# KyleVanMeter/MVOLPS

Measured on AMD Instinct MI355X. Metric: simplex_pivots_per_s, higher is better.
Workload: dtype f64

## Files before the change

### mvolps_amd/csrc/engine.cpp

```cpp
#include <hip/hip_runtime.h>

#include <cmath>
#include <cstdio>
#include <cstdlib>
#include <cstring>
#include <atomic>
#include <functional>
#include <limits>
#include <map>
#include <mutex>
#include <tuple>
#include <unordered_map>
#include <unordered_set>
#include <vector>

#include "engine.hpp"

struct DevMatrix {
  int m0 = 0, n = 0, lda = 0;
  double *plain = nullptr, *packed = nullptr;
  int *len = nullptr;
  std::vector<const void *> rows;
  ~DevMatrix() {
    if (packed && packed != plain) (void)hipFree(packed);
// ... 1033 lines not shown
  if (J.parm.it_lim > 8 && J.try_fused) J.batch = std::min(J.parm.it_lim, 256);
}

static void job_enqueue(Context &c, SolveJob &J) {
  mvx_prob *P = J.P;
  SolveCtx &sc = *J.sc;
  const int m = P->m, n = P->n;
  J.ev_used = 0;
  if (J.mode == SolveJob::FINAL) {
    launch_export(sc.d_ctl, sc.d_stage, m, n, 1, sc.stream);
    stage_copy_async(sc, P);
    return;
  }
  if (J.mode == SolveJob::PHASE1) {
    for (int k = 0; k < J.pb; k++) {
      launch_p1_head(sc.d_ctl, sc.stream);
      launch_p1_fix(sc.d_ctl, n, sc.stream);
      launch_p1_select(sc.d_ctl, sc.stream);
      launch_update(sc.d_ctl, m + 1, n, sc.stream);
    }
    launch_export(sc.d_ctl, sc.d_stage, m, n, 0, sc.stream);
    stage_copy_async(sc, P);
    return;
  }
  const int batch = J.batch;
  if (J.profiled && c.ev_pool.size() < (size_t)2 * batch + 4) {
    size_t old = c.ev_pool.size();
    c.ev_pool.resize((size_t)2 * batch + 4);
    for (size_t k = old; k < c.ev_pool.size(); k++) HIPCHECK(hipEventCreate(&c.ev_pool[k]));
  }
  const int remaining = (J.parm.it_lim >= 0) ? std::max(0, J.parm.it_lim - J.seen_pivots) : (1 << 30);
  auto ev = [&]() {
    if (J.profiled) HIPCHECK(hipEventRecord(c.ev_pool[J.ev_used++], sc.stream));
  };
  int depth;
  if (J.try_fused) depth = std::max(0, std::min(batch, remaining));
  else depth = std::max(1, std::min(batch, remaining));
  auto body = [&](int m_grid) {
    if (J.try_fused) {
      PersistPlan pl;
      if (depth > 0 && !J.profiled && J.resident && !(J.cluster && !g_cluster_broken.load()) && persist_plan(c, P, &pl) && ensure_persist(c, sc, P, pl)) {
        launch_select(sc.d_ctl, sc.stream);
        launch_update(sc.d_ctl, m_grid, n, sc.stream, 1, 1);
        HIPCHECK(hipMemcpyAsync(sc.p_backup, P->slab, P->slab_bytes, hipMemcpyDeviceToDevice, sc.stream));
        HIPCHECK(hipMemcpyAsync(sc.d_pctl, sc.d_ctl, sizeof(Ctl), hipMemcpyDeviceToDevice, sc.stream));
        HIPCHECK(hipMemcpyAsync(sc.d_ppw, sc.d_pw[0], (size_t)P->ld * 8, hipMemcpyDeviceToDevice, sc.stream));
        HIPCHECK(hipMemcpyAsync(sc.d_ppw + P->ld, sc.d_pw[1], (size_t)P->ld * 8, hipMemcpyDeviceToDevice, sc.stream));
        const int head_stride = 4;
        HIPCHECK(hipMemsetAsync(sc.d_pcand, 0, (size_t)2 * pl.nw * head_stride * 8, sc.stream));
        const int steps = 1 << 24;
        if (launch_persist(sc.d_ctl, sc.d_pcand, sc.d_pmsg, sc.d_pabort, (unsigned long long *)(sc.d_pabort + 16), P->m, pl.cpw, pl.nw, sc.p_msg_words, steps, head_stride, sc.stream) == 0) {
          J.persist_queued = true;
          g_persist_launches++;
          launch_select(sc.d_ctl, sc.stream);
          launch_update(sc.d_ctl, m_grid, n, sc.stream, 1, 1);
        } else {
          g_persist_broken = true;
        }
      } else {
        const size_t e_generic = J.ev_used;
        if (J.profiled) J.ev_used += 2;
        if (depth > 0) {
          const bool cl = J.cluster && !g_cluster_broken.load();
          if (!cl) launch_pboot(J.cargs, sc.stream);
          bool first = true;
          const int kc = cl ? std::max(1, std::min(J.chain0, chain_cluster_kmax(m, n))) : std::max(1, J.chain);
          auto chain_launch = [&](int steps) {
            J.cargs.kmax = steps;
            J.cargs.boot = first ? 1 : 0;
            first = false;
            J.cargs.tagbase = sc.xtag;
            sc.xtag += 128;
            if (launch_chain(J.cargs, sc.stream) != 0) g_cluster_broken.store(true);
            g_cluster_launches++;
          };
          for (int left = depth; left > 0;) {
            const int steps = std::min(kc, left);
            if (cl) chain_launch(steps);
            else
              for (int t = 0; t < steps; t++) launch_pstep(J.cargs, t, sc.stream);
            ev();
            launch_fbc3(J.cargs, steps, sc.stream);
            ev();
            launch_fpatch(J.cargs, steps, sc.stream);
            left -= steps;
          }
          if (J.parm.it_lim >= 0 && depth >= remaining && !cl) launch_pc(J.cargs, 0, sc.stream);
        }
        launch_select(sc.d_ctl, sc.stream);
        if (J.profiled) HIPCHECK(hipEventRecord(c.ev_pool[e_generic], sc.stream));
        launch_update(sc.d_ctl, m_grid, n, sc.stream, 1, 1);
        if (J.profiled) HIPCHECK(hipEventRecord(c.ev_pool[e_generic + 1], sc.stream));
      }
    } else if (J.try_dfused) {
      launch_select(sc.d_ctl, sc.stream);
      launch_update(sc.d_ctl, m_grid, n, sc.stream, 1, 1);
      if (depth > 1) {
        launch_dboot(sc.d_ctl, n, sc.stream);
        launch_db(sc.d_ctl, m_grid, n, sc.stream);
        for (int k = 0; k < depth - 1; k++) {
          launch_da(sc.d_ctl, n, sc.stream);
          launch_db(sc.d_ctl, m_grid, n, sc.stream);
        }
      }
    } else {
      for (int k = 0; k < depth; k++) {
        launch_dsel(sc.d_ctl, m, n, sc.stream);
        launch_select(sc.d_ctl, sc.stream);
        ev();
        launch_update(sc.d_ctl, m_grid, n, sc.stream, 1, 1);
        ev();
      }
    }
    launch_export(sc.d_ctl, sc.d_stage, m_grid, n, 0, sc.stream);
    stage_copy_async(sc, P);
  };
  body(m);
}

static bool job_finalize(SolveJob &J) {
  mvx_prob *P = J.P;
  SolveCtx &sc = *J.sc;
  const Ctl &snap = J.snap;
  const unsigned char *s = sc.h_stage;
  const double *beta = (const double *)(s + sizeof(Ctl));
  const double *dj = beta + (P->m_cap + 1);
  const int *bv = (const int *)(dj + P->ld);
  const int *nv = bv + (P->m_cap + 1);
  const int *nf = nv + P->ld;
  P->beta.assign(beta, beta + P->m + 1);
  P->dj.assign(dj, dj + P->n + 1);
  P->bvar.assign(bv, bv + P->m + 1);
  P->nvar.assign(nv, nv + P->n + 1);
  P->nflag.assign(nf, nf + P->n + 1);
  rebuild_pos(P);
  P->sol_fresh = true;
  P->fresh_rows = -1;
  float ms = 0.f;
  HIPCHECK(hipEventElapsedTime(&ms, sc.ev_a, sc.ev_b));
  P->last_ms = ms;
  P->it_cnt += snap.it_cnt;
  P->bland_cnt += snap.n_bland;
  P->pert_cnt += snap.n_pert;
  P->hint_dual = false;
  switch (J.done) {
    case D_OPT: P->status = MVX_OPT; J.rc = 0; break;
    case D_UNBND: P->status = MVX_UNBND; J.rc = 0; break;
    case D_NOFEAS: P->status = MVX_NOFEAS; J.rc = 0; break;
    case D_ITLIM:
      P->status = (snap.phase == PH_PRIMAL2) ? MVX_FEAS : MVX_INFEAS;
      J.rc = MVX_EITLIM;
      break;
    default: P->status = MVX_UNDEF; J.rc = MVX_EFAIL; break;
  }
  return true;
}

static bool job_collect(Context &c, SolveJob &J) {
  SolveCtx &sc = *J.sc;
  Ctl &snap = J.snap;
  if (J.persist_queued) {
    J.persist_queued = false;
    if (sc.h_pabort[0]) {
      mvx_prob *P = J.P;
      g_persist_broken = true;
      g_persist_aborts++;
      std::fprintf(stderr, "mvx: resident-tableau launch aborted (workgroups not co-resident in time); using the two-kernel path from now on\n");
// ... 2077 lines not shown
```

### mvolps_amd/csrc/kernels.hip

```cpp
#include <hip/hip_runtime.h>

#include <cmath>
#include <cstdlib>

#include "kernel_common.hpp"

namespace mvx {

template <int MODE>
__device__ __forceinline__ bool cand_better(const Cand &a, const Cand &b) {
  if (a.idx == 0) return false;
  if (b.idx == 0) return true;
  if (MODE == 0) {
    if (a.k1 > b.k1) return true;
    if (a.k1 < b.k1) return false;
    return a.idx < b.idx;
  } else {
    if (a.k1 < b.k1) return true;
    if (a.k1 > b.k1) return false;
    if (a.k2 > b.k2) return true;
    if (a.k2 < b.k2) return false;
    return a.idx < b.idx;
  }
}

template <int MODE>
__device__ __forceinline__ Cand wave_best(Cand c) {
#pragma unroll
  for (int off = 32; off > 0; off >>= 1) {
    Cand o;
    o.k1 = __shfl_down(c.k1, off, 64);
    o.k2 = __shfl_down(c.k2, off, 64);
    o.idx = __shfl_down(c.idx, off, 64);
    o.aux = __shfl_down(c.aux, off, 64);
    if (cand_better<MODE>(o, c)) c = o;
  }
  return c;
}

template <int MODE>
__device__ Cand block_best(Cand c, Cand *lds) {
  const int lane = TIDX & 63, wid = TIDX >> 6, nw = (int)blockDim.x >> 6;
  c = wave_best<MODE>(c);
  __syncthreads();
  if (lane == 0) lds[wid] = c;
  __syncthreads();
  if (wid == 0) {
    Cand r = (lane < nw) ? lds[lane] : Cand{0.0, 0.0, 0, 0};
    r = wave_best<MODE>(r);
    if (lane == 0) lds[16] = r;
  }
  __syncthreads();
  return lds[16];
}

template <int MODE>
__device__ __forceinline__ Cand wave_bcast_best(Cand b) {
  b = wave_best<MODE>(b);
  Cand r;
  r.k1 = __shfl(b.k1, 0, 64);
  r.k2 = __shfl(b.k2, 0, 64);
  r.idx = __shfl(b.idx, 0, 64);
  r.aux = __shfl(b.aux, 0, 64);
  return r;
}

__device__ __forceinline__ int rl_i(int x, int l) { return __builtin_amdgcn_readlane(x, l); }
__device__ __forceinline__ double rl_d(double x, int l) {
  const int lo = __builtin_amdgcn_readlane(__double2loint(x), l), hi = __builtin_amdgcn_readlane(__double2hiint(x), l);
  return __hiloint2double(hi, lo);
}
__device__ __forceinline__ double wave_max_f64(double v) {
  const int ilo = __double2loint(-INFINITY), ihi = __double2hiint(-INFINITY);
#define WMAX_STEP(CTRL, RMASK)                                                                            \
  {                                                                                                       \
    const int lo = __builtin_amdgcn_update_dpp(ilo, __double2loint(v), CTRL, RMASK, 0xf, false);          \
    const int hi = __builtin_amdgcn_update_dpp(ihi, __double2hiint(v), CTRL, RMASK, 0xf, false);          \
    v = fmax(v, __hiloint2double(hi, lo));                                                                \
  }
  WMAX_STEP(0x111, 0xf)
  WMAX_STEP(0x112, 0xf)
  WMAX_STEP(0x114, 0xf)
  WMAX_STEP(0x118, 0xf)
  WMAX_STEP(0x142, 0xa)
// ... 2549 lines not shown
      A.drowk[xf][0] = z;
      A.pwk[xf][0] = 1.0;
    }
  }
  if (lead) {
    c->pc_n = g;
    if (g > 0) {
      c->phase = PH_PRIMAL2;
      c->pc_itlim = end_itlim ? 1 : 0;
    }
  }
}

__device__ void chain_commit(const ChainArgs &A, Ctl *c, int nch) {
  __shared__ int s_cp[KCH], s_cq[KCH], s_ck[KCH], s_rf[KCH], s_cf[KCH], s_R[KCH], s_C[KCH];
  const int t = TIDX;
  const bool on = (t < nch);
  int kind = 0, p = 0, q = 0;
  if (on) {
    kind = c->ch_kind[t];
    p = c->ch_p[t];
    q = c->ch_q[t];
    s_ck[t] = kind;
    s_cp[t] = p;
    s_cq[t] = q;
    s_R[t] = (kind == ST_PIVOT) ? c->bvar[p] : 0;
    s_C[t] = (kind == ST_PIVOT) ? c->nvar[q] : 0;
  }
  __syncthreads();
  bool lastrow = true, lastcol = true, lastflag = true;
  if (on) {
    int rf = t, cf = t;
    for (int u = t - 1; u >= 0; u--) {
      if (s_ck[u] != ST_PIVOT) continue;
      if (s_cp[u] == p) rf = u;
      if (s_cq[u] == q) cf = u;
    }
    s_rf[t] = rf;
    s_cf[t] = cf;
    for (int u = t + 1; u < nch; u++) {
      if (s_cq[u] == q) lastflag = false;
      if (s_ck[u] != ST_PIVOT) continue;
      if (s_cp[u] == p) lastrow = false;
      if (s_cq[u] == q) lastcol = false;
    }
  }
  __syncthreads();
  if (t == 0) {
    for (int u = 0; u < nch; u++) {
      if (s_ck[u] != ST_PIVOT) continue;
      const int a = s_rf[u], b = s_cf[u];
      const int kv = s_R[a];
      s_R[a] = s_C[b];
      s_C[b] = kv;
    }
  }
  __syncthreads();
  if (on) {
    if (kind == ST_PIVOT) {
      if (lastrow) {
        c->bvar[p] = s_R[s_rf[t]];
        A.blb[p] = c->ch_elb[t];
        A.bub[p] = c->ch_eub[t];
      }
      if (lastcol) {
        c->nvar[q] = s_C[s_cf[t]];
        A.nlb[q] = c->ch_llb[t];
        A.nub[q] = c->ch_lub[t];
      }
    }
    if (lastflag) A.nflag[q] = c->ch_lf[t];
  }
  if (t == 0) {
    const int piv_n = c->ch_cnt[nch - 1];
    c->it_cnt += piv_n;
    c->n_flips += nch - piv_n;
    c->n_bulk++;
    if (c->budget > 0) c->budget -= piv_n;
    c->stall = c->ch_stall[nch - 1];
    c->pc_epoch++;
  }
}

typedef const double __attribute__((address_space(4))) *kconst_f64;
template <int TR, int NT>
__global__ __launch_bounds__(256) void k_fbc3(const ChainArgs A) {
  __shared__ double s_cq[KCH][TR];
  Ctl *const c = A.c;
  if (c->done != D_RUN || c->fstate != F_RUN) return;
  const int nch = c->pc_n;
  if (nch == 0) return;
  const int n = A.n;
  const size_t ld = (size_t)A.ld;
  const int j0 = 2 * ((int)blockIdx.x * 256 + TIDX);
  const int i0 = 1 + (int)blockIdx.y * TR;
  const int xf = nch & 1;
  const bool act = (j0 <= n);
  const int jc = act ? j0 : 0;
  double *base = A.T + (size_t)i0 * ld + jc;
  double2 v[TR];
#pragma unroll
  for (int r = 0; r < TR; r++) v[r] = ld2<NT>(reinterpret_cast<const double2 *>(base + (size_t)r * ld));
  unsigned flips = 0;
  for (int l = 0; l < nch; l++) flips |= (c->ch_kind[l] == ST_FLIP) ? (1u << l) : 0u;
  for (int e = TIDX; e < nch * TR; e += 256) {
    const int l = e / TR, r = e % TR;
    s_cq[l][r] = ((flips >> l) & 1u) ? 0.0 : A.colq0[(size_t)l * A.cstride + i0 + r];
  }
  __syncthreads();
  const double *sp = A.srow0 + jc;
  const double *zp = A.zeros + jc;
  for (int l0 = 0; l0 < nch; l0 += 4) {
    double2 s4[4];
#pragma unroll
    for (int k = 0; k < 4; k++) {
      const int lk = (l0 + k < nch) ? l0 + k : nch - 1;
      s4[k] = *reinterpret_cast<const double2 *>(((flips >> lk) & 1u) ? zp : sp + (size_t)lk * A.sstride);
    }
#pragma unroll
    for (int k = 0; k < 4; k++) {
      if (l0 + k < nch) {
#pragma unroll
        for (int r = 0; r < TR; r++) {
          const double ci = s_cq[l0 + k][r];
          asm("v_fma_f64 %0, -%1, %2, %0" : "+v"(v[r].x) : "v"(ci), "v"(s4[k].x));
          asm("v_fma_f64 %0, -%1, %2, %0" : "+v"(v[r].y) : "v"(ci), "v"(s4[k].y));
        }
      }
    }
  }
  if (act) {
    if (j0 == 0) {
#pragma unroll
      for (int r = 0; r < TR; r++) base[(size_t)r * ld + 1] = v[r].y;
    } else {
#pragma unroll
      for (int r = 0; r < TR; r++) st2<NT>(reinterpret_cast<double2 *>(base + (size_t)r * ld), v[r]);
    }
    if (blockIdx.y == 0) {
      *reinterpret_cast<double2 *>(A.T + j0) = *reinterpret_cast<const double2 *>(A.drowk[xf] + j0);
      const double2 w = *reinterpret_cast<const double2 *>(A.pwk[xf] + j0);
      *reinterpret_cast<double2 *>(A.pw[0] + j0) = w;
      *reinterpret_cast<double2 *>(A.pw[1] + j0) = w;
    }
  }
  if (blockIdx.x == 0 && blockIdx.y == 0) chain_commit(A, c, nch);
}

__global__ __launch_bounds__(256) void k_fpatch(const ChainArgs A, int kmax) {
  __shared__ int s_kind[KCH], s_p[KCH], s_q[KCH];
  __shared__ double s_piv[KCH], s_ip[KCH], s_xq[KCH], s_delta[KCH], s_u[KCH];
  Ctl *const c = A.c;
  if (c->done != D_RUN || c->fstate != F_RUN) return;
  const int nch = c->pc_n;
  if (nch == 0) return;
  const int m = A.m, n = A.n;
  const size_t ld = (size_t)A.ld;
  const int job = (int)blockIdx.y, x = (int)blockIdx.x * 256 + TIDX;
  const int jk = (job < kmax) ? 0 : (job < 2 * kmax) ? 1 : 2;
  const int l = (jk == 0) ? job : (jk == 1) ? job - kmax : -1;
  bool live = (jk == 2) || (l < nch && c->ch_kind[l < nch ? l : 0] == ST_PIVOT);
  const int span = (jk == 0) ? n : (jk == 1) ? m : A.mcap1 - 1;
  if ((int)blockIdx.x * 256 > span) live = false;
  if (live) {
    const int lp = (l >= 0) ? c->ch_p[l] : 0, lq = (l >= 0) ? c->ch_q[l] : 0;
    if (TIDX < KCH) {
      const int t = (TIDX < nch) ? TIDX : nch - 1;
      const int kind = c->ch_kind[t];
      const double piv = c->ch_piv[t];
      s_kind[TIDX] = kind;
      s_p[TIDX] = c->ch_p[t];
      s_q[TIDX] = c->ch_q[t];
      s_piv[TIDX] = piv;
      s_ip[TIDX] = (kind == ST_PIVOT) ? xdiv(1.0, piv) : 0.0;
      s_xq[TIDX] = c->ch_xq[t];
      s_delta[TIDX] = c->ch_delta[t];
      s_u[TIDX] = (jk == 0) ? A.colq0[(size_t)t * A.cstride + lp] : A.srow0[(size_t)t * A.sstride + (jk == 1 ? lq : 0)];
    }
    const int xc = (x >= 1 && x <= span) ? x : 1;
    double op[KCH];
#pragma unroll
    for (int t = 0; t < KCH; t++) {
      const int tc = (t < nch) ? t : nch - 1;
      op[t] = (jk == 0) ? A.srow0[(size_t)tc * A.sstride + xc] : A.colq0[(size_t)tc * A.cstride + xc];
    }
    double *dst = (jk == 0) ? A.T + (size_t)lp * ld + xc : A.T + (size_t)xc * ld + (jk == 1 ? lq : 0);
    double val = (jk == 2) ? *dst : 0.0;
    __syncthreads();
    const int i = (jk == 0) ? lp : xc, j = (jk == 0) ? xc : (jk == 1) ? lq : 0;
    const int l0 = (jk == 2) ? 0 : l;
#pragma unroll
    for (int t = 0; t < KCH; t++) {
      if (t >= l0 && t < nch) {
        const double ci = (jk == 0) ? s_u[t] : op[t], sj = (jk == 0) ? op[t] : s_u[t];
        if (s_kind[t] == ST_FLIP) {
          if (j == 0) val = fma(ci, s_delta[t], val);
        } else if (i == s_p[t]) {
          val = (j == s_q[t]) ? s_ip[t] : (j == 0) ? s_xq[t] - sj : -sj;
        } else if (j == s_q[t]) {
          val = xdiv(ci, s_piv[t]);
        } else {
          val = fma(-ci, sj, val);
        }
      }
    }
    if (x >= 1 && x <= span) {
      if (jk != 2 || x <= m) *dst = val;
      if (jk == 2) A.betab[x] = val;
    }
  }
}

__device__ __forceinline__ bool row_violation(double beta, double lb, double ub, double tol, double &viol, int &up) {
  viol = 0.0;
  up = 0;
  if (lb > -INFINITY && beta < lb - tol * (1.0 + fabs(lb))) viol = lb - beta;
  if (ub < INFINITY && beta > ub + tol * (1.0 + fabs(ub))) {
    viol = beta - ub;
    up = 1;
  }
  return viol > 0.0;
}

__device__ __forceinline__ bool dual_ratio_col(double a, double d, int f, int to_upper, double tp, int j, Cand &x) {
  if (f == MVX_NS) return false;
  const double aa = to_upper ? -a : a;
  double r;
  if (aa > tp && (f == MVX_NL || f == MVX_NF)) r = (f == MVX_NF) ? fabs(d) : (d < 0.0 ? -d : 0.0);
  else if (aa < -tp && (f == MVX_NU || f == MVX_NF)) r = (f == MVX_NF) ? fabs(d) : (d > 0.0 ? d : 0.0);
  else return false;
  const double mag = fabs(a);
  x = Cand{xdiv(r, mag), mag, j, 0};
  return true;
}

__global__ __launch_bounds__(DA_THREADS) void k_dboot(Ctl *c) {
  __shared__ Cand lds[17];
  const bool lead = (blockIdx.x == 0 && TIDX == 0);
  if (c->done != D_RUN || c->phase != PH_DUAL || c->stall >= c->stall_limit || c->perturbed) {
    if (lead) c->fstate = F_OFF;
    return;
  }
  const int a = c->curA & 1, m = c->m, n = c->n;
  const size_t ld = (size_t)c->ld;
  const double *T = c->T, *w = c->dwx[a];
  const double tol = c->tol_bnd;
  Cand rb{0.0, 0.0, 0, 0};
  for (int i = 1 + TIDX; i <= m; i += DA_THREADS) {
    double viol;
    int up;
    if (row_violation(T[(size_t)i * ld], c->blb[i], c->bub[i], tol, viol, up)) {
      Cand x{xdiv(viol * viol, w[i]), 0.0, i, up};
      if (cand_better<0>(x, rb)) rb = x;
    }
  }
  rb = block_best<0>(rb, lds);
  const int p2 = rb.idx, p2_up = rb.aux;
  const int j = (int)blockIdx.x * DA_THREADS + TIDX;
  Cand best{0.0, 0.0, 0, 0};
  if (p2 && j >= 1 && j <= n) {
    Cand x{0.0, 0.0, 0, 0};
    if (dual_ratio_col(T[(size_t)p2 * ld + j], c->sgn * T[j], c->nflag[j], p2_up, c->tol_piv, j, x)) best = x;
  }
  __syncthreads();
  best = block_best<1>(best, lds);
  if (TIDX == 0) c->pp[a][blockIdx.x] = best;
  if (lead) {
    c->p_nextx[a] = p2;
    c->p_up_nextx[a] = p2_up;
    c->fstate = F_RUN_DUAL;
    c->step = ST_NONE;
    c->curB = a ^ 1;
    c->npbd = (int)gridDim.x;
  }
}

__global__ __launch_bounds__(DA_THREADS) void k_da(Ctl *c) {
  __shared__ Cand lds[17];
  const int done = c->done, fstate = c->fstate, cur = c->curA, budget = c->budget;
  const int stall = c->stall, stall_limit = c->stall_limit;
  const int npb = c->npbd, m = c->m, n = c->n;
  const size_t ld = (size_t)c->ld;
  double *const T = c->T;
  double *const srow = c->srow;
  const int *const nflag = c->nflag;
  const double *const colq = c->colqx[cur];
  const double *const betac = c->betac[cur];
  const Cand *const pp = c->pp[cur];
  Cand *const ppn = c->pp[cur ^ 1];
  const double *const dwc = c->dwx[cur & 1];
  double *const dwn = c->dwx[(cur & 1) ^ 1];
  const double sgn = c->sgn, tol_bnd = c->tol_bnd, tol_piv = c->tol_piv;
  const int p = c->p_nextx[cur & 1], p_up = c->p_up_nextx[cur & 1];
// ... 466 lines not shown
                   int slot_stride, int max_steps, int head_stride, hipStream_t s) {
  static size_t attr_bytes = 0;
  const size_t lds = persist_lds_bytes(m, cpw);
  if (lds > attr_bytes) {
    if (hipFuncSetAttribute(reinterpret_cast<const void *>(k_persist), hipFuncAttributeMaxDynamicSharedMemorySize, (int)lds) != hipSuccess) {
      (void)hipGetLastError();
      return -1;
    }
    attr_bytes = lds;
  }
  PersistArgs a;
  a.ctl = d_ctl; a.head = head; a.slot = slot; a.abort_flag = abort_flag; a.dbg = dbg;
  a.cpw = cpw; a.nw = nw; a.slot_stride = slot_stride; a.max_steps = max_steps;
  a.head_stride = head_stride;
  hipLaunchKernelGGL(k_persist, dim3((unsigned)nw), dim3(256), lds, s, a);
  return hipGetLastError() == hipSuccess ? 0 : -1;
}


static int g_tr = 0, g_hot = 1, g_nt = -1;
void set_tuning(int tr, int hot, int nt) {
  g_tr = (tr == 4 || tr == 8 || tr == 16 || tr == 32) ? tr : 0;
  g_hot = hot ? 1 : 0;
  g_nt = (nt >= 0 && nt <= 2) ? nt : -1;
}
static int pick_nt(int m, int n) {
  if (g_nt >= 0) return g_nt;
  const size_t bytes = (size_t)(m + 1) * (size_t)((n + 1 + LD_ALIGN - 1) / LD_ALIGN * LD_ALIGN) * 8;
  if (bytes > NT_THRESHOLD_BYTES) return 1;
  return (bytes >= WT_MIN_BYTES && bytes <= WT_MAX_BYTES) ? 2 : 0;
}
static int pick_tr(int m, int n) {
  if (g_tr) return g_tr;
  const long tiles = ((n + 2) / 2 + 255) / 256;
  if ((long)((m + 15) / 16) * tiles >= 2048) return 16;
  if ((long)((m + 7) / 8) * tiles >= 2048) return 8;
  return 4;
}
int fused_npb(int n) { return (n + 1 + 255) / 256; }
int fused_nrb_max(int m) { return (m + 3) / 4; }
int chain_ncb(int n) { return fused_npb(n); }
int chain_nrb(int m) { return (m + 255) / 256; }
void launch_pboot(const ChainArgs &a, hipStream_t s) {
  hipLaunchKernelGGL(k_pboot, dim3(a.ncb > a.nrb ? a.ncb : a.nrb), dim3(256), 0, s, a);
}
void launch_pstep(const ChainArgs &a, int g, hipStream_t s) {
  hipLaunchKernelGGL(k_pc, dim3(a.nrb), dim3(256), 0, s, a, g);
  hipLaunchKernelGGL(k_pr, dim3(a.ncb), dim3(256), 0, s, a, g);
}
void launch_pc(const ChainArgs &a, int g, hipStream_t s) { hipLaunchKernelGGL(k_pc, dim3(a.nrb), dim3(256), 0, s, a, g); }
int chain_cluster_nw(int m, int n) {
  const int span = m > n ? m : n;
  int nw = (span + 255) / 256;
  if (nw > 32) nw = 32;
  return nw < 1 ? 1 : nw;
}
int chain_cluster_kmax(int m, int n) {
  const int nw = chain_cluster_nw(m, n), tt = nw * 256;
  const int cpt = (n + tt - 1) / tt, rpt = (m + tt - 1) / tt;
  if (cpt > 2 || rpt > 2) return 0;
  const int per_step = (cpt > 1 || rpt > 1 ? 4 : 2) * 256 * 8;
  const int k = (140 * 1024) / per_step;
  return k > KCH ? KCH : k;
}
int launch_chain(const ChainArgs &a, hipStream_t s) {
  const int tt = a.nw * 256;
  const int cpt = (a.n + tt - 1) / tt, rpt = (a.m + tt - 1) / tt;
  const bool wide = (cpt > 1 || rpt > 1);
  const size_t lds = (size_t)(a.kmax > 0 ? a.kmax : 1) * (wide ? 4 : 2) * 256 * 8;
  static size_t attr1 = 0, attr2 = 0;
  size_t &attr = wide ? attr2 : attr1;
  const void *fn = wide ? reinterpret_cast<const void *>(k_chain<2, 2>) : reinterpret_cast<const void *>(k_chain<1, 1>);
  if (lds > attr) {
    if (hipFuncSetAttribute(fn, hipFuncAttributeMaxDynamicSharedMemorySize, (int)lds) != hipSuccess) {
      (void)hipGetLastError();
      return -1;
    }
    attr = lds;
  }
  if (wide) hipLaunchKernelGGL((k_chain<2, 2>), dim3(8 * a.nw), dim3(256), lds, s, a);
  else hipLaunchKernelGGL((k_chain<1, 1>), dim3(8 * a.nw), dim3(256), lds, s, a);
  return 0;
}
void launch_fpatch(const ChainArgs &a, int steps, hipStream_t s) {
  const int span = a.mcap1 > a.n + 1 ? a.mcap1 : a.n + 1;
  hipLaunchKernelGGL(k_fpatch, dim3((span + 255) / 256, 2 * steps + 1), dim3(256), 0, s, a, steps);
}
void launch_fbc3(const ChainArgs &a, int steps, hipStream_t s) {
  const int m = a.m, n = a.n;
  const int pairs = (n + 2) / 2;
  int tr = pick_tr(m, n);
  if (tr > 16) tr = 16;
  if (!g_tr && tr == 16 && steps >= 12) tr = 8;
  const int nt = pick_nt(m, n);
  dim3 grid((pairs + 255) / 256, (m + tr - 1) / tr);
#define FBC2_CASE(TR_, NT_) \
  if (tr == TR_ && nt == NT_) { hipLaunchKernelGGL((k_fbc3<TR_, NT_>), grid, dim3(256), 0, s, a); return; }
  FBC2_CASE(16, 0) FBC2_CASE(16, 1) FBC2_CASE(16, 2) FBC2_CASE(8, 0) FBC2_CASE(8, 1) FBC2_CASE(8, 2) FBC2_CASE(4, 0) FBC2_CASE(4, 1) FBC2_CASE(4, 2)
#undef FBC2_CASE
  std::abort();
}
void launch_dboot(Ctl *d_ctl, int n, hipStream_t s) { hipLaunchKernelGGL(k_dboot, dim3((n + DA_THREADS) / DA_THREADS), dim3(DA_THREADS), 0, s, d_ctl); }
void launch_da(Ctl *d_ctl, int n, hipStream_t s) { hipLaunchKernelGGL(k_da, dim3((n + DA_THREADS) / DA_THREADS), dim3(DA_THREADS), 0, s, d_ctl); }
void launch_db(Ctl *d_ctl, int m, int n, hipStream_t s) {
  const int pairs = (n + 2) / 2;
  const int tr = pick_tr(m, n);
  const int nt = pick_nt(m, n);
  dim3 grid((pairs + 255) / 256, (m + tr - 1) / tr);
#define DB_CASE(TR_, NT_) \
  if (tr == TR_ && nt == NT_) { hipLaunchKernelGGL((k_fb<TR_, 1, NT_, 1>), grid, dim3(256), 0, s, d_ctl); return; }
  DB_CASE(16, 0) DB_CASE(16, 1) DB_CASE(8, 0) DB_CASE(8, 1) DB_CASE(4, 0) DB_CASE(4, 1) DB_CASE(32, 0) DB_CASE(32, 1)
  DB_CASE(16, 2) DB_CASE(8, 2) DB_CASE(4, 2) DB_CASE(32, 2)
#undef DB_CASE
  std::abort();
}
int launch_dsel(Ctl *d_ctl, int m, int n, hipStream_t s, int slots) {
  static int state = -1;
  if (state < 0) {
    const char *e = std::getenv("MVX_DSEL");
    if (e && e[0] == '0') state = 0;
    else if (hipFuncSetAttribute(reinterpret_cast<const void *>(k_dsel), hipFuncAttributeMaxDynamicSharedMemorySize, (int)DSEL_LDS) == hipSuccess) state = 1;
    else {
      (void)hipGetLastError();
      state = 0;
    }
  }
  if (state != 1 || m > 1024 || n > 1024) return 0;
  hipLaunchKernelGGL(k_dsel, dim3(1, 1, slots), dim3(1024), DSEL_LDS, s, d_ctl);
  return 1;
}
void launch_select(Ctl *d_ctl, hipStream_t s, int slots) {
  BatchQueue q{};
  hipLaunchKernelGGL(k_select, dim3(1, 1, slots), dim3(1024), 0, s, d_ctl, q);
}
void launch_select_queue(Ctl *d_ctl, const BatchQueue &q, hipStream_t s, int slots) {
  hipLaunchKernelGGL(k_select, dim3(1, 1, slots), dim3(1024), 0, s, d_ctl, q);
}
void launch_update(Ctl *d_ctl, int m, int n, hipStream_t s, int slots, int chained, int busy_slots) {
  const int pairs = (n + 2) / 2;
  const long tiles = (pairs + 255) / 256;
  const long work = busy_slots > 0 ? std::min(busy_slots, slots) : slots;
  int tr = ((long)((m + 16) / 16) * tiles * work >= 2048) ? 16 : ((long)((m + 8) / 8) * tiles * work >= 2048) ? 8 : 4;
  static const int tr_cap = std::getenv("MVX_UPD_TR") ? std::atoi(std::getenv("MVX_UPD_TR")) : 4;
  if (slots > 1 && chained && tr > tr_cap) tr = tr_cap >= 16 ? 16 : tr_cap >= 8 ? 8 : 4;
  dim3 grid((unsigned)tiles, (m + tr) / tr, slots);
  const int nt = (tr == 16) ? pick_nt(m, n) : 0;
  if (nt == 1) hipLaunchKernelGGL((k_update<16, 1>), grid, dim3(256), 0, s, d_ctl, chained);
  else if (nt == 2) hipLaunchKernelGGL((k_update<16, 2>), grid, dim3(256), 0, s, d_ctl, chained);
  else if (tr == 16) hipLaunchKernelGGL((k_update<16, 0>), grid, dim3(256), 0, s, d_ctl, chained);
  else if (tr == 8) hipLaunchKernelGGL((k_update<8, 0>), grid, dim3(256), 0, s, d_ctl, chained);
  else hipLaunchKernelGGL((k_update<4, 0>), grid, dim3(256), 0, s, d_ctl, chained);
}
void launch_p1_head(Ctl *d_ctl, hipStream_t s) { hipLaunchKernelGGL(k_p1_head, dim3(1), dim3(1024), 0, s, d_ctl); }
void launch_p1_select(Ctl *d_ctl, hipStream_t s) { hipLaunchKernelGGL(k_p1_select, dim3(1), dim3(1024), 0, s, d_ctl); }
__global__ __launch_bounds__(64) void k_scatter_ctl(Ctl *dst, const Ctl *src, const int *idx, int count) {
  const int t = (int)blockIdx.x;
  if (t >= count) return;
  const unsigned *s = reinterpret_cast<const unsigned *>(&src[t]);
  unsigned *d = reinterpret_cast<unsigned *>(&dst[idx[t]]);
  for (int w = TIDX; w < (int)(sizeof(Ctl) / 4); w += 64) d[w] = s[w];
}
void launch_scatter_ctl(Ctl *dst, const Ctl *src, const int *idx, int count, hipStream_t s) {
  hipLaunchKernelGGL(k_scatter_ctl, dim3(count), dim3(64), 0, s, dst, src, idx, count);
}
__global__ __launch_bounds__(256) void k_copy_many(CopyBatch b) {
  const CopyJob j = b.jobs[blockIdx.y];
  const uint4 *__restrict__ src = reinterpret_cast<const uint4 *>(j.src);
  uint4 *__restrict__ dst = reinterpret_cast<uint4 *>(j.dst);
  const size_t n = j.bytes >> 4;
  constexpr int U = 8;
  for (size_t base = (size_t)blockIdx.x * (256 * U); base < n; base += (size_t)gridDim.x * (256 * U)) {
    uint4 v[U];
#pragma unroll
    for (int u = 0; u < U; u++) {
      const size_t i = base + (size_t)u * 256 + TIDX;
      if (i < n) v[u] = src[i];
    }
#pragma unroll
    for (int u = 0; u < U; u++) {
      const size_t i = base + (size_t)u * 256 + TIDX;
// ... 41 lines not shown
```

### mvolps_amd/csrc/mvx_internal.hpp

```cpp
#pragma once

#include <cstddef>
#include <cstdint>
#include <memory>
#include <string>
#include <vector>

#include <hip/hip_runtime_api.h>

#include "../../include/mvx.h"

struct DevMatrix;
namespace mvx {

constexpr int ROWCOMB_CHUNK = 64;
constexpr int LD_ALIGN = 32;
constexpr int ROW_SLACK = 64;
constexpr double DEGEN_TOL = 1e-9;
constexpr double PERT_EPS = 1e-6;
constexpr size_t NT_THRESHOLD_BYTES = (size_t)320 << 20;
constexpr size_t WT_MIN_BYTES = (size_t)96 << 20, WT_MAX_BYTES = (size_t)272 << 20;
constexpr int KCH = 32;
constexpr int DCH_MAX = 8;
constexpr int DA_THREADS = 1024;
// ... 284 lines not shown
  const int *rowcol;
  const int *nbcol;
  const double *rowlb;
  const int *extra;
  int m, n, ld, k;
};

#define DEL_BATCH 8
struct DelRowsArgs {
  double *T;
  int *bvar, *nvar;
  double *blb, *bub;
  const int *src;
  const int *del;
  int first, nmove, m_old, nrs, n, ld;
};
struct DelManyDesc {
  double *T;
  int *bvar, *nvar;
  double *blb, *bub;
  unsigned long long o_src, o_del;
  int first, nmove, m_old, nrs, n, ld;
};

#define CONF_WAVES 4
struct ConflictArgs {
  const double *At;
  const double *Ar;
  const double *rlo, *rhi;
  const double *clo, *chi;
  const int *flags;
  double *rowinfo;
  unsigned long long *adj;
  int n, m0, ldm, ldn, W, pad;
};

#define LS_GROUP 8
struct LsRec {
  double gain;
  unsigned long long key;
};
struct LsArgs {
  const double *At;
  const double *Ar;
  const double *rlo, *rhi;
  const double *clo, *chi;
  const double *c;
  const int *flags;
  const double *xin;
  double *x;
  double *r;
  double *obj, *obj0;
  int *moves, *ok, *done;
  LsRec *rec;
  double sg;
  int n, m0, ldm, ldn, count, pad;
};

struct SetbHandle {
  double *T, *blb, *bub, *nlb, *nub;
  int *nflag;
  int ld, m;
  int e0, e1;
  int s0, s1;
};
struct SetbEntry {
  double lb, ub;
  int idx, flag;
};
struct SetbShift {
  double delta;
  int jj, pad;
};

void set_tuning(int tr, int hot, int nt);
int fused_npb(int n);
int fused_nrb_max(int m);
int chain_ncb(int n);
int chain_nrb(int m);
void launch_pboot(const ChainArgs &, hipStream_t);
void launch_pstep(const ChainArgs &, int g, hipStream_t);
void launch_pc(const ChainArgs &, int g, hipStream_t);
void launch_fbc3(const ChainArgs &, int steps, hipStream_t);
void launch_fpatch(const ChainArgs &, int steps, hipStream_t);
int launch_chain(const ChainArgs &, hipStream_t);
int chain_cluster_nw(int m, int n);
int chain_cluster_kmax(int m, int n);
void launch_dboot(Ctl *, int n, hipStream_t);
void launch_da(Ctl *, int n, hipStream_t);
void launch_db(Ctl *, int m, int n, hipStream_t);
void launch_select(Ctl *, hipStream_t, int slots = 1);
int launch_dsel(Ctl *, int m, int n, hipStream_t, int slots = 1);
void launch_select_queue(Ctl *, const BatchQueue &q, hipStream_t, int slots);
void launch_update(Ctl *, int m, int n, hipStream_t, int slots = 1, int chained = 0, int busy_slots = 0);
void launch_p1_head(Ctl *, hipStream_t);
void launch_p1_select(Ctl *, hipStream_t);
void launch_p1_fix(Ctl *, int n, hipStream_t);
void launch_scatter_ctl(Ctl *dst, const Ctl *src, const int *idx, int count, hipStream_t);
void launch_copy_many(const CopyBatch &b, hipStream_t);
void launch_gmi(const GmiArgs &a, hipStream_t);
void launch_classify(const ClsArgs &a, hipStream_t);
void launch_penalty(const PenArgs &a, hipStream_t);
void launch_round(const RndArgs &a, hipStream_t);
void launch_rcfix(const RcArgs &a, hipStream_t);
void launch_prop(const PropArgs &a, hipStream_t);
void launch_divepick(const DiveArgs &a, hipStream_t);
void launch_objrow(const ObjNode *nodes, int n, int count, hipStream_t);
void launch_pumpobj(const PumpArgs &a, hipStream_t);
void launch_cutgram(const CutGramArgs &a, hipStream_t);
void launch_cutrows(const CutRowsArgs &a, hipStream_t);
void launch_delrows(const DelRowsArgs &a, hipStream_t);
void launch_delrows_many(const DelManyDesc *hs, const unsigned char *base, int handles, int max_ld, hipStream_t);
void launch_conflict(const ConflictArgs &a, hipStream_t);
void launch_lsact(const LsArgs &a, int final, hipStream_t);
void launch_lsiter(const LsArgs &a, hipStream_t);
void launch_setbnds(const SetbHandle *hs, const SetbEntry *es, const SetbShift *ss, int handles, hipStream_t);
void launch_refresh_select(Ctl *, const int *tflag, int var, hipStream_t);
size_t persist_lds_bytes(int m, int cpw);
int persist_max_cpw();
int persist_slot_words(int m_cap);
int launch_persist(Ctl *, unsigned long long *head, unsigned long long *slot, int *abort_flag, unsigned long long *dbg, int m, int cpw, int nw,
                   int slot_stride, int max_steps, int head_stride, hipStream_t);
void launch_rowcomb(Ctl *, int m, int n, int respect_done, hipStream_t);
void launch_shift_nonbasic(double *T, int ld, int m, int jj, double delta, hipStream_t);
void launch_set_basic_bounds(double *blb, double *bub, int i, double lb, double ub, hipStream_t);
void launch_set_nonbasic(double *nlb, double *nub, int *nflag, int j, double lb, double ub, int flag, hipStream_t);
void launch_add_rows(double *T, int ld, int n, int *bvar, double *blb, double *bub, int *nvar, int first, int nrs, int m_new,
                     hipStream_t);
void launch_export(Ctl *, unsigned char *stage, int m, int n, int force, hipStream_t, int slots = 1, size_t slot_stride = 0);

using RowPtr = std::shared_ptr<std::vector<double>>;

template <class T>
class CowVec {
  std::shared_ptr<std::vector<T>> p_ = std::make_shared<std::vector<T>>();

public:
  const T &operator[](size_t i) const { return (*p_)[i]; }
  size_t size() const { return p_->size(); }
  bool empty() const { return p_->empty(); }
  const std::vector<T> &get() const { return *p_; }
  std::vector<T> &mut() {
    if (p_.use_count() != 1) p_ = std::make_shared<std::vector<T>>(*p_);
    return *p_;
  }
};

class RowList {
  std::shared_ptr<std::vector<RowPtr>> head_ = std::make_shared<std::vector<RowPtr>>();
  std::vector<RowPtr> tail_;

public:
  size_t size() const { return head_->size() + tail_.size(); }
  const RowPtr &operator[](size_t i) const { return i < head_->size() ? (*head_)[i] : tail_[i - head_->size()]; }
  size_t tail_size() const { return tail_.size(); }
  void push_back(RowPtr r) { tail_.push_back(std::move(r)); }
  void set(size_t i, RowPtr r) {
    if (i >= head_->size()) {
      tail_[i - head_->size()] = std::move(r);
      return;
    }
    if (head_.use_count() != 1) head_ = std::make_shared<std::vector<RowPtr>>(*head_);
    (*head_)[i] = std::move(r);
  }
  void resize(size_t n) {
    if (n >= head_->size()) {
      tail_.resize(n - head_->size());
// ... 88 lines not shown
```

Before: 57720.

## Fuse pivot patch kernel into bulk chain update and interleave patch blocks

Merges the separate fpatch kernel into k_fbc3 by giving the launch a 1-D grid that interleaves bulk-update tiles with patch blocks. Bulk tiles skip writing the pivot rows and columns that patch blocks own, so the two can run concurrently without a kernel boundary. It also double-buffers the step-row loads in groups of four, computes flip masks with ballots instead of a serial loop, caps TR at 8, and alternates the tile order between launches. The aim is to remove a launch and a serialization point per chain segment. The price is more complex ownership logic: any error in the masks would corrupt the tableau.

```diff
diff --git a/mvolps_amd/csrc/engine.cpp b/mvolps_amd/csrc/engine.cpp
--- a/mvolps_amd/csrc/engine.cpp
+++ b/mvolps_amd/csrc/engine.cpp
@@ -1139,7 +1139,6 @@
             ev();
             launch_fbc3(J.cargs, steps, sc.stream);
             ev();
-            launch_fpatch(J.cargs, steps, sc.stream);
             left -= steps;
           }
           if (J.parm.it_lim >= 0 && depth >= remaining && !cl) launch_pc(J.cargs, 0, sc.stream);
diff --git a/mvolps_amd/csrc/kernels.hip b/mvolps_amd/csrc/kernels.hip
--- a/mvolps_amd/csrc/kernels.hip
+++ b/mvolps_amd/csrc/kernels.hip
@@ -1,5 +1,6 @@
 #include <hip/hip_runtime.h>
 
+#include <atomic>
 #include <cmath>
 #include <cstdlib>
 
@@ -2715,133 +2716,201 @@
   }
 }
 
-typedef const double __attribute__((address_space(4))) *kconst_f64;
+struct PatchLds {
+  int kind[KCH], p[KCH], q[KCH];
+  double piv[KCH], ip[KCH], xq[KCH], delta[KCH], u[KCH];
+};
+__device__ __forceinline__ void fbc3_patch(const ChainArgs &A, Ctl *c, int kmax, int job, int xb, PatchLds &L) {
+  const int t32 = TIDX & (KCH - 1);
+  const int kind = c->ch_kind[t32], chp = c->ch_p[t32], chq = c->ch_q[t32];
+  const double piv = c->ch_piv[t32], xq = c->ch_xq[t32], delta = c->ch_delta[t32];
+  const int done = c->done, fstate = c->fstate, nch = c->pc_n;
+  if (done != D_RUN || fstate != F_RUN || nch <= 0) return;
+  const int m = A.m, n = A.n;
+  const size_t ld = (size_t)A.ld;
+  const int x = xb * 256 + TIDX;
+  const int jk = (job < kmax) ? 0 : (job < 2 * kmax) ? 1 : 2;
+  const int l = (jk == 0) ? job : (jk == 1) ? job - kmax : -1;
+  const int lc = (l >= 0 && l < nch) ? l : 0;
+  bool live = (jk == 2) || (l < nch && __builtin_amdgcn_readlane(kind, lc) == ST_PIVOT);
+  const int span = (jk == 0) ? n : (jk == 1) ? m : A.mcap1 - 1;
+  if (xb * 256 > span) live = false;
+  if (!live) return;
+  const int lp = (l >= 0) ? __builtin_amdgcn_readlane(chp, lc) : 0, lq = (l >= 0) ? __builtin_amdgcn_readlane(chq, lc) : 0;
+  if (TIDX < KCH) {
+    const int t = (TIDX < nch) ? TIDX : nch - 1;
+    L.kind[TIDX] = kind;
+    L.p[TIDX] = chp;
+    L.q[TIDX] = chq;
+    L.piv[TIDX] = piv;
+    L.ip[TIDX] = (kind == ST_PIVOT) ? xdiv(1.0, piv) : 0.0;
+    L.xq[TIDX] = xq;
+    L.delta[TIDX] = delta;
+    L.u[TIDX] = (jk == 0) ? A.colq0[(size_t)t * A.cstride + lp] : A.srow0[(size_t)t * A.sstride + (jk == 1 ? lq : 0)];
+  }
+  const int xc = (x >= 1 && x <= span) ? x : 1;
+  double op[KCH];
+#pragma unroll
+  for (int t = 0; t < KCH; t++) {
+    const int tc = (t < nch) ? t : nch - 1;
+    op[t] = (jk == 0) ? A.srow0[(size_t)tc * A.sstride + xc] : A.colq0[(size_t)tc * A.cstride + xc];
+  }
+  double *dst = (jk == 0) ? A.T + (size_t)lp * ld + xc : A.T + (size_t)xc * ld + (jk == 1 ? lq : 0);
+  double val = (jk == 2) ? *dst : 0.0;
+  __syncthreads();
+  const int i = (jk == 0) ? lp : xc, j = (jk == 0) ? xc : (jk == 1) ? lq : 0;
+  const int l0 = (jk == 2) ? 0 : l;
+#pragma unroll
+  for (int t = 0; t < KCH; t++) {
+    if (t >= l0 && t < nch) {
+      const double ci = (jk == 0) ? L.u[t] : op[t], sj = (jk == 0) ? op[t] : L.u[t];
+      if (L.kind[t] == ST_FLIP) {
+        if (j == 0) val = fma(ci, L.delta[t], val);
+      } else if (i == L.p[t]) {
+        val = (j == L.q[t]) ? L.ip[t] : (j == 0) ? L.xq[t] - sj : -sj;
+      } else if (j == L.q[t]) {
+        val = xdiv(ci, L.piv[t]);
+      } else {
+        val = fma(-ci, sj, val);
+      }
+    }
+  }
+  if (x >= 1 && x <= span) {
+    if (jk != 2 || x <= m) *dst = val;
+    if (jk == 2) A.betab[x] = val;
+  }
+}
+
+constexpr int FBG = 4;
+static_assert(KCH % FBG == 0, "whole groups: the last group's filling steps need rows of their own in the staging area");
+template <int TR>
+__device__ __forceinline__ void fbc3_apply(double2 (&v)[TR], const double2 (&s)[FBG], const double *cq, int l0) {
+#pragma unroll
+  for (int k = 0; k < FBG; k++) {
+#pragma unroll
+    for (int r = 0; r < TR; r++) {
+      const double ci = cq[(l0 + k) * TR + r];
+      asm("v_fma_f64 %0, -%1, %2, %0" : "+v"(v[r].x) : "v"(ci), "v"(s[k].x));
+      asm("v_fma_f64 %0, -%1, %2, %0" : "+v"(v[r].y) : "v"(ci), "v"(s[k].y));
+    }
+  }
+}
+struct BulkGrid {
+  int kmax, ncb, ntile, npatch, every;
+  int rev;
+};
 template <int TR, int NT>
-__global__ __launch_bounds__(256) void k_fbc3(const ChainArgs A) {
-  __shared__ double s_cq[KCH][TR];
+__global__ __launch_bounds__(256) void k_fbc3(const ChainArgs A, const BulkGrid G) {
+  constexpr int NS = (KCH * TR + 255) / 256;
+  __shared__ double s_cq[NS * 256];
+  __shared__ PatchLds s_patch;
   Ctl *const c = A.c;
-  if (c->done != D_RUN || c->fstate != F_RUN) return;
-  const int nch = c->pc_n;
-  if (nch == 0) return;
+  int tile = -1, patch = -1;
+  {
+    const int b = (int)blockIdx.x;
+    if (G.every > 0) {
+      const int g = b / (G.every + 1), rm = b - g * (G.every + 1);
+      if (g >= G.npatch) tile = b - G.npatch;
+      else if (rm == G.every) patch = g;
+      else tile = g * G.every + rm;
+    } else if (b < G.ntile) {
+      tile = b;
+    } else {
+      patch = b - G.ntile;
+    }
+  }
+  if (patch >= 0) {
+    const int njobs = 2 * G.kmax + 1;
+    fbc3_patch(A, c, G.kmax, patch % njobs, patch / njobs, s_patch);
+    return;
+  }
+  const int kind = c->ch_kind[TIDX & (KCH - 1)], chp = c->ch_p[TIDX & (KCH - 1)], chq = c->ch_q[TIDX & (KCH - 1)];
+  const int done = c->done, fstate = c->fstate, nch = c->pc_n;
+  if (done != D_RUN || fstate != F_RUN || nch <= 0) return;
+  const int bx = tile % G.ncb, by = G.rev ? G.ntile / G.ncb - 1 - tile / G.ncb : tile / G.ncb;
   const int n = A.n;
   const size_t ld = (size_t)A.ld;
-  const int j0 = 2 * ((int)blockIdx.x * 256 + TIDX);
-  const int i0 = 1 + (int)blockIdx.y * TR;
+  const int j0 = 2 * (bx * 256 + TIDX);
+  const int i0 = 1 + by * TR;
   const int xf = nch & 1;
   const bool act = (j0 <= n);
   const int jc = act ? j0 : 0;
+  double cs[NS];
+#pragma unroll
+  for (int u = 0; u < NS; u++) {
+    const int e = TIDX + u * 256, ec = (e < nch * TR) ? e : 0;
+    cs[u] = A.colq0[(size_t)(ec / TR) * A.cstride + i0 + ec % TR];
+  }
+  const unsigned zsteps = (unsigned)__ballot((TIDX & 63) >= nch || kind == ST_FLIP);
+  const double *const srow = A.srow0 + jc;
+  const ptrdiff_t zrow = A.zeros - A.srow0, sstride = (ptrdiff_t)A.sstride;
+  auto rowpair = [&](int l) {
+    const int lk = (l < KCH) ? l : KCH - 1;
+    return *reinterpret_cast<const double2 *>(srow + (((zsteps >> lk) & 1u) ? zrow : lk * sstride));
+  };
+  double2 sa[FBG], sb[FBG];
+#pragma unroll
+  for (int k = 0; k < FBG; k++) sa[k] = rowpair(k);
+#pragma unroll
+  for (int k = 0; k < FBG; k++) sb[k] = rowpair(FBG + k);
   double *base = A.T + (size_t)i0 * ld + jc;
   double2 v[TR];
 #pragma unroll
   for (int r = 0; r < TR; r++) v[r] = ld2<NT>(reinterpret_cast<const double2 *>(base + (size_t)r * ld));
-  unsigned flips = 0;
-  for (int l = 0; l < nch; l++) flips |= (c->ch_kind[l] == ST_FLIP) ? (1u << l) : 0u;
-  for (int e = TIDX; e < nch * TR; e += 256) {
-    const int l = e / TR, r = e % TR;
-    s_cq[l][r] = ((flips >> l) & 1u) ? 0.0 : A.colq0[(size_t)l * A.cstride + i0 + r];
+#pragma unroll
+  for (int u = 0; u < NS; u++) {
+    const int e = TIDX + u * 256;
+    s_cq[e] = ((zsteps >> ((e / TR) & (KCH - 1))) & 1u) ? 0.0 : cs[u];
+  }
+  const bool pivot = (TIDX & 63) < nch && kind == ST_PIVOT;
+  unsigned rowown = 0;
+#pragma unroll
+  for (int r = 0; r < TR; r++) rowown |= __ballot(pivot && chp == i0 + r) ? (1u << r) : 0u;
+  bool own_x = (j0 == 0), own_y = false;
+  {
+    const int jw = 2 * (bx * 256 + (TIDX & ~63));
+    unsigned long long cm = __ballot(pivot && (unsigned)(chq - jw) < 128u);
+    while (cm) {
+      const int l = __ffsll((long long)cm) - 1;
+      cm &= cm - 1;
+      const int ql = __builtin_amdgcn_readlane(chq, l);
+      own_x |= (ql == j0);
+      own_y |= (ql == j0 + 1);
+    }
   }
   __syncthreads();
-  const double *sp = A.srow0 + jc;
-  const double *zp = A.zeros + jc;
-  for (int l0 = 0; l0 < nch; l0 += 4) {
-    double2 s4[4];
-#pragma unroll
-    for (int k = 0; k < 4; k++) {
-      const int lk = (l0 + k < nch) ? l0 + k : nch - 1;
-      s4[k] = *reinterpret_cast<const double2 *>(((flips >> lk) & 1u) ? zp : sp + (size_t)lk * A.sstride);
-    }
-#pragma unroll
-    for (int k = 0; k < 4; k++) {
-      if (l0 + k < nch) {
-#pragma unroll
-        for (int r = 0; r < TR; r++) {
-          const double ci = s_cq[l0 + k][r];
-          asm("v_fma_f64 %0, -%1, %2, %0" : "+v"(v[r].x) : "v"(ci), "v"(s4[k].x));
-          asm("v_fma_f64 %0, -%1, %2, %0" : "+v"(v[r].y) : "v"(ci), "v"(s4[k].y));
-        }
-      }
-    }
-  }
+  fbc3_apply<TR>(v, sa, s_cq, 0);
+  int l0 = FBG;
+  for (; l0 + FBG < nch; l0 += 2 * FBG) {
+#pragma unroll
+    for (int k = 0; k < FBG; k++) sa[k] = rowpair(l0 + FBG + k);
+    fbc3_apply<TR>(v, sb, s_cq, l0);
+#pragma unroll
+    for (int k = 0; k < FBG; k++) sb[k] = rowpair(l0 + 2 * FBG + k);
+    fbc3_apply<TR>(v, sa, s_cq, l0 + FBG);
+  }
+  if (l0 < nch) fbc3_apply<TR>(v, sb, s_cq, l0);
   if (act) {
-    if (j0 == 0) {
-#pragma unroll
-      for (int r = 0; r < TR; r++) base[(size_t)r * ld + 1] = v[r].y;
+    if (!own_x && !own_y) {
+#pragma unroll
+      for (int r = 0; r < TR; r++)
+        if (!((rowown >> r) & 1u)) st2<NT>(reinterpret_cast<double2 *>(base + (size_t)r * ld), v[r]);
     } else {
 #pragma unroll
-      for (int r = 0; r < TR; r++) st2<NT>(reinterpret_cast<double2 *>(base + (size_t)r * ld), v[r]);
-    }
-    if (blockIdx.y == 0) {
+      for (int r = 0; r < TR; r++) {
+        if ((rowown >> r) & 1u) continue;
+        if (!own_x) base[(size_t)r * ld] = v[r].x;
+        if (!own_y) base[(size_t)r * ld + 1] = v[r].y;
+      }
+    }
+    if (by == 0) {
       *reinterpret_cast<double2 *>(A.T + j0) = *reinterpret_cast<const double2 *>(A.drowk[xf] + j0);
       const double2 w = *reinterpret_cast<const double2 *>(A.pwk[xf] + j0);
       *reinterpret_cast<double2 *>(A.pw[0] + j0) = w;
       *reinterpret_cast<double2 *>(A.pw[1] + j0) = w;
     }
   }
-  if (blockIdx.x == 0 && blockIdx.y == 0) chain_commit(A, c, nch);
-}
-
-__global__ __launch_bounds__(256) void k_fpatch(const ChainArgs A, int kmax) {
-  __shared__ int s_kind[KCH], s_p[KCH], s_q[KCH];
-  __shared__ double s_piv[KCH], s_ip[KCH], s_xq[KCH], s_delta[KCH], s_u[KCH];
-  Ctl *const c = A.c;
-  if (c->done != D_RUN || c->fstate != F_RUN) return;
-  const int nch = c->pc_n;
-  if (nch == 0) return;
-  const int m = A.m, n = A.n;
-  const size_t ld = (size_t)A.ld;
-  const int job = (int)blockIdx.y, x = (int)blockIdx.x * 256 + TIDX;
-  const int jk = (job < kmax) ? 0 : (job < 2 * kmax) ? 1 : 2;
-  const int l = (jk == 0) ? job : (jk == 1) ? job - kmax : -1;
-  bool live = (jk == 2) || (l < nch && c->ch_kind[l < nch ? l : 0] == ST_PIVOT);
-  const int span = (jk == 0) ? n : (jk == 1) ? m : A.mcap1 - 1;
-  if ((int)blockIdx.x * 256 > span) live = false;
-  if (live) {
-    const int lp = (l >= 0) ? c->ch_p[l] : 0, lq = (l >= 0) ? c->ch_q[l] : 0;
-    if (TIDX < KCH) {
-      const int t = (TIDX < nch) ? TIDX : nch - 1;
-      const int kind = c->ch_kind[t];
-      const double piv = c->ch_piv[t];
-      s_kind[TIDX] = kind;
-      s_p[TIDX] = c->ch_p[t];
-      s_q[TIDX] = c->ch_q[t];
-      s_piv[TIDX] = piv;
-      s_ip[TIDX] = (kind == ST_PIVOT) ? xdiv(1.0, piv) : 0.0;
-      s_xq[TIDX] = c->ch_xq[t];
-      s_delta[TIDX] = c->ch_delta[t];
-      s_u[TIDX] = (jk == 0) ? A.colq0[(size_t)t * A.cstride + lp] : A.srow0[(size_t)t * A.sstride + (jk == 1 ? lq : 0)];
-    }
-    const int xc = (x >= 1 && x <= span) ? x : 1;
-    double op[KCH];
-#pragma unroll
-    for (int t = 0; t < KCH; t++) {
-      const int tc = (t < nch) ? t : nch - 1;
-      op[t] = (jk == 0) ? A.srow0[(size_t)tc * A.sstride + xc] : A.colq0[(size_t)tc * A.cstride + xc];
-    }
-    double *dst = (jk == 0) ? A.T + (size_t)lp * ld + xc : A.T + (size_t)xc * ld + (jk == 1 ? lq : 0);
-    double val = (jk == 2) ? *dst : 0.0;
-    __syncthreads();
-    const int i = (jk == 0) ? lp : xc, j = (jk == 0) ? xc : (jk == 1) ? lq : 0;
-    const int l0 = (jk == 2) ? 0 : l;
-#pragma unroll
-    for (int t = 0; t < KCH; t++) {
-      if (t >= l0 && t < nch) {
-        const double ci = (jk == 0) ? s_u[t] : op[t], sj = (jk == 0) ? op[t] : s_u[t];
-        if (s_kind[t] == ST_FLIP) {
-          if (j == 0) val = fma(ci, s_delta[t], val);
-        } else if (i == s_p[t]) {
-          val = (j == s_q[t]) ? s_ip[t] : (j == 0) ? s_xq[t] - sj : -sj;
-        } else if (j == s_q[t]) {
-          val = xdiv(ci, s_piv[t]);
-        } else {
-          val = fma(-ci, sj, val);
-        }
-      }
-    }
-    if (x >= 1 && x <= span) {
-      if (jk != 2 || x <= m) *dst = val;
-      if (jk == 2) A.betab[x] = val;
-    }
-  }
+  if (tile == 0) chain_commit(A, c, nch);
 }
 
 __device__ __forceinline__ bool row_violation(double beta, double lb, double ub, double tol, double &viol, int &up) {
@@ -3474,20 +3543,25 @@
   else hipLaunchKernelGGL((k_chain<1, 1>), dim3(8 * a.nw), dim3(256), lds, s, a);
   return 0;
 }
-void launch_fpatch(const ChainArgs &a, int steps, hipStream_t s) {
-  const int span = a.mcap1 > a.n + 1 ? a.mcap1 : a.n + 1;
-  hipLaunchKernelGGL(k_fpatch, dim3((span + 255) / 256, 2 * steps + 1), dim3(256), 0, s, a, steps);
-}
 void launch_fbc3(const ChainArgs &a, int steps, hipStream_t s) {
   const int m = a.m, n = a.n;
   const int pairs = (n + 2) / 2;
   int tr = pick_tr(m, n);
   if (tr > 16) tr = 16;
-  if (!g_tr && tr == 16 && steps >= 12) tr = 8;
+  if (!g_tr && tr > 8) tr = 8;
   const int nt = pick_nt(m, n);
-  dim3 grid((pairs + 255) / 256, (m + tr - 1) / tr);
+  const int span = a.mcap1 > n + 1 ? a.mcap1 : n + 1;
+  BulkGrid g;
+  g.kmax = steps;
+  g.ncb = (pairs + 255) / 256;
+  g.ntile = g.ncb * ((m + tr - 1) / tr);
+  g.npatch = (2 * steps + 1) * ((span + 255) / 256);
+  g.every = g.ntile / g.npatch;
+  static std::atomic<unsigned> launches{0};
+  g.rev = (steps >= 4) ? (int)(launches.fetch_add(1, std::memory_order_relaxed) & 1u) : 0;
+  const dim3 grid(g.ntile + g.npatch);
 #define FBC2_CASE(TR_, NT_) \
-  if (tr == TR_ && nt == NT_) { hipLaunchKernelGGL((k_fbc3<TR_, NT_>), grid, dim3(256), 0, s, a); return; }
+  if (tr == TR_ && nt == NT_) { hipLaunchKernelGGL((k_fbc3<TR_, NT_>), grid, dim3(256), 0, s, a, g); return; }
   FBC2_CASE(16, 0) FBC2_CASE(16, 1) FBC2_CASE(16, 2) FBC2_CASE(8, 0) FBC2_CASE(8, 1) FBC2_CASE(8, 2) FBC2_CASE(4, 0) FBC2_CASE(4, 1) FBC2_CASE(4, 2)
 #undef FBC2_CASE
   std::abort();
diff --git a/mvolps_amd/csrc/mvx_internal.hpp b/mvolps_amd/csrc/mvx_internal.hpp
--- a/mvolps_amd/csrc/mvx_internal.hpp
+++ b/mvolps_amd/csrc/mvx_internal.hpp
@@ -390,7 +390,6 @@
 void launch_pstep(const ChainArgs &, int g, hipStream_t);
 void launch_pc(const ChainArgs &, int g, hipStream_t);
 void launch_fbc3(const ChainArgs &, int steps, hipStream_t);
-void launch_fpatch(const ChainArgs &, int steps, hipStream_t);
 int launch_chain(const ChainArgs &, hipStream_t);
 int chain_cluster_nw(int m, int n);
 int chain_cluster_kmax(int m, int n);
```

Result: faster. 63120, median of 6 (+9.4%).
